# RenYurui/Global-Flow-Local-Attention

Hardware: AMD Instinct MI355X
Metric: images/sec (fwd+bwd) PoseGenerator 256x176 attn_layer=2,3 -- feature-warping hot path (higher is better)
Workload: dtype f32 (FC products: 2-term f16 splits exact to 2^-24 on f16 MFMA, f32 accumulate)

## Files before the change

global_flow_local_attention_amd/csrc/patch_mfma.hip:

```cpp
#include "gfla_common.h"
#include "patch_mfma.h"
#include "rs_taps.h"

namespace gfla {

typedef float pm_f32x16 __attribute__((ext_vector_type(16)));

struct PatchEntry {
  int q;
  float v;
};

constexpr int kPmStatSlots = 32;
constexpr int kPmTile = 32;
constexpr int kPmSub = 8;
constexpr int kPmChannels = 128;
constexpr int kPmMaxNB = 6;
constexpr int kPmGPitch = 33;

struct PmLayout {
  int64_t ntiles, table_bytes, rows_bytes, total;
};
static PmLayout pm_layout(int64_t B, int64_t HW, int entries) {
  PmLayout L;
  L.ntiles = ceil_div(HW, kPmTile);
  L.table_bytes = ((B * L.ntiles * kPmTile * entries * (int64_t)sizeof(PatchEntry)) + 255) & ~(int64_t)255;
  L.rows_bytes = ((B * L.ntiles * (int64_t)sizeof(int2)) + 255) & ~(int64_t)255;
  L.total = L.table_bytes + L.rows_bytes + 256;
  return L;
}

__device__ __forceinline__ unsigned pm_stat_total(const unsigned *stat) {
  unsigned tot = 0;
#pragma unroll
  for (int i = 0; i < kPmStatSlots; ++i) tot += stat[i];
  return tot;
}

__device__ __forceinline__ int pm_safe_int(float v) {
  return (int)fminf(fmaxf(v, -1048576.f), 1048576.f);
}

__device__ __forceinline__ void pm_store_tile_rows(int lo, int hi, int2 *slot, unsigned *stat) {
  __shared__ int s_lo[4], s_hi[4];
#pragma unroll
  for (int m = 32; m >= 1; m >>= 1) {
    lo = min(lo, __shfl_xor(lo, m));
    hi = max(hi, __shfl_xor(hi, m));
  }
  if ((threadIdx.x & 63) == 0) {
    s_lo[threadIdx.x >> 6] = lo;
    s_hi[threadIdx.x >> 6] = hi;
  }
  __syncthreads();
  if (threadIdx.x == 0) {
    const int l = min(min(s_lo[0], s_lo[1]), min(s_lo[2], s_lo[3])), h = max(max(s_hi[0], s_hi[1]), max(s_hi[2], s_hi[3]));
    *slot = make_int2(l, h);
    if (h >= l) atomicAdd(stat + (blockIdx.x + blockIdx.y * gridDim.x) % kPmStatSlots, (unsigned)(h - l + 1));
  }
}

struct Fold {
  int r_lo, r_hi, s_lo, s_hi, ty, tx;
  bool canonical;
};
__device__ __forceinline__ Fold pm_fold(int r, int s, int y0, int x0, int P, int Hs, int Ws) {
  Fold f;
  const int yy = y0 + r, xx = x0 + s;
  f.r_lo = f.r_hi = r;
  f.s_lo = f.s_hi = s;
  f.canonical = true;
  if (yy <= 0) {
    f.r_lo = 0;
    f.canonical = f.canonical && (yy == 0 || r == P - 1);
  } else if (yy >= Hs - 1) {
    f.r_hi = P - 1;
    f.canonical = f.canonical && (yy == Hs - 1 || r == 0);
  }
  if (xx <= 0) {
    f.s_lo = 0;
    f.canonical = f.canonical && (xx == 0 || s == P - 1);
  } else if (xx >= Ws - 1) {
    f.s_hi = P - 1;
    f.canonical = f.canonical && (xx == Ws - 1 || s == 0);
  }
  f.ty = clampi(yy, 0, Hs - 1);
  f.tx = clampi(xx, 0, Ws - 1);
  return f;
}

template <int K>
struct AggTaps {
  float fx0, fy0;
  int xf, yf, x0, y0;
  bool dense;
  __device__ __forceinline__ float dx(int t) const { return (fx0 + (float)(t - K / 2)) + (float)xf; }
  __device__ __forceinline__ float dy(int t) const { return (fy0 + (float)(t - K / 2)) + (float)yf; }
  __device__ __forceinline__ float ax(int t) const { const float d = dx(t); return d - floorf(d); }
  __device__ __forceinline__ float ay(int t) const { const float d = dy(t); return d - floorf(d); }
  __device__ __forceinline__ void init(float fx, float fy, int x, int y) {
    fx0 = fx, fy0 = fy, xf = x, yf = y;
    dense = true;
    x0 = y0 = 0;
#pragma unroll
    for (int t = 0; t < K; ++t) {
      const int ix = (int)floorf(dx(t)), iy = (int)floorf(dy(t));
      if (t == 0) x0 = ix, y0 = iy;
      dense = dense && (ix == x0 + t) && (iy == y0 + t);
    }
  }
};

template <int K>
__global__ __launch_bounds__(256) void agg_patch_table_kernel(const float *__restrict__ flow,
                                                             const float *__restrict__ attn,
                                                             PatchEntry *__restrict__ table,
                                                             int2 *__restrict__ tile_rows,
                                                             unsigned *__restrict__ stat, int H, int W, int Hs, int Ws,
                                                             int ntiles) {
  constexpr int P = K + 1, E = P * P, KK = K * K;
  static_assert(E % 2 == 0, "entries are written two at a time");
  typedef int i32x4 __attribute__((ext_vector_type(4)));
  const int64_t b = blockIdx.y;
  const int HW = H * W;
  const int tile = blockIdx.x * 8 + (threadIdx.x >> 5), pl = threadIdx.x & 31;
  if (tile >= ntiles) return;
  const int p = tile * kPmTile + pl;
  const float inv_kk = 1.f / (float)KK;
  int lo = 0x7fffffff, hi = -1;
  i32x4 *out = reinterpret_cast<i32x4 *>(table + ((b * ntiles + tile) * kPmTile + pl) * (int64_t)E);
  bool dense = false;
  AggTaps<K> tp;
  if (p < HW) {
    const int yf = p / W, xf = p - yf * W;
    tp.init(flow[(b * 2 + 0) * HW + p], flow[(b * 2 + 1) * HW + p], xf, yf);
    dense = tp.dense;
  }
  if (dense) {
    const int y0 = pm_safe_int((float)tp.y0), x0 = pm_safe_int((float)tp.x0);
    lo = clampi(y0, 0, Hs - 1);
    hi = clampi(y0 + K, 0, Hs - 1);
    float a[KK];
    const float *at = attn + b * (int64_t)KK * HW + p;
#pragma unroll
    for (int t = 0; t < KK; ++t) a[t] = at[(int64_t)t * HW] * inv_kk;
    float ax[K], ay[K];
#pragma unroll
    for (int t = 0; t < K; ++t) {
      ax[t] = tp.ax(t);
      ay[t] = tp.ay(t);
    }
    float v[P][P];
#pragma unroll
    for (int r = 0; r < P; ++r) {
#pragma unroll
      for (int q = 0; q < P; ++q) v[r][q] = 0.f;
#pragma unroll
      for (int j = 0; j < K; ++j) {
        float wrow = 0.f;
        if (r < K) wrow += a[r * K + j] * (1.f - ay[r]);
        if (r > 0) wrow += a[(r - 1) * K + j] * ay[r - 1];
        v[r][j] += wrow * (1.f - ax[j]);
        v[r][j + 1] += wrow * ax[j];
      }
    }
    int clo[P], chi[P], rlo[P], rhi[P], tx[P], ty[P];
    bool ccan[P], rcan[P];
#pragma unroll
    for (int i = 0; i < P; ++i) {
      const int xx = x0 + i, yy = y0 + i;
      clo[i] = chi[i] = rlo[i] = rhi[i] = i;
      ccan[i] = rcan[i] = true;
      if (xx <= 0) {
        clo[i] = 0;
        ccan[i] = xx == 0 || i == P - 1;
      } else if (xx >= Ws - 1) {
        chi[i] = P - 1;
        ccan[i] = xx == Ws - 1 || i == 0;
      }
      if (yy <= 0) {
        rlo[i] = 0;
        rcan[i] = yy == 0 || i == P - 1;
      } else if (yy >= Hs - 1) {
        rhi[i] = P - 1;
        rcan[i] = yy == Hs - 1 || i == 0;
      }
      tx[i] = clampi(xx, 0, Ws - 1);
      ty[i] = clampi(yy, 0, Hs - 1);
    }
    float cf[P][P];
#pragma unroll
    for (int r = 0; r < P; ++r)
#pragma unroll
      for (int q = 0; q < P; ++q) {
        float acc = 0.f;
#pragma unroll
        for (int q2 = 0; q2 < P; ++q2) acc += (q2 >= clo[q] && q2 <= chi[q]) ? v[r][q2] : 0.f;
        cf[r][q] = acc;
      }
#pragma unroll
    for (int r = 0; r < P; ++r)
#pragma unroll
      for (int q = 0; q < P; q += 2) {
        float acc0 = 0.f, acc1 = 0.f;
#pragma unroll
        for (int r2 = 0; r2 < P; ++r2) {
          const bool in = r2 >= rlo[r] && r2 <= rhi[r];
          acc0 += in ? cf[r2][q] : 0.f;
          acc1 += in ? cf[r2][q + 1] : 0.f;
        }
        const bool c0 = rcan[r] && ccan[q], c1 = rcan[r] && ccan[q + 1];
        i32x4 e;
        e.x = c0 ? (ty[r] << 16) | tx[q] : -1;
        e.y = c0 ? __float_as_int(acc0) : 0;
        e.z = c1 ? (ty[r] << 16) | tx[q + 1] : -1;
        e.w = c1 ? __float_as_int(acc1) : 0;
        out[(r * P + q) >> 1] = e;
      }
  } else {
    const i32x4 none = {-1, 0, -1, 0};
#pragma unroll
    for (int e = 0; e < E / 2; ++e) out[e] = none;
  }
#pragma unroll
  for (int msk = 16; msk >= 1; msk >>= 1) {
    lo = min(lo, __shfl_xor(lo, msk));
    hi = max(hi, __shfl_xor(hi, msk));
  }
  if (pl == 0) {
    tile_rows[b * ntiles + tile] = make_int2(lo, hi);
    if (hi >= lo) atomicAdd(stat + (tile + (int)b * ntiles) % kPmStatSlots, (unsigned)(hi - lo + 1));
  }
}

template <int K>
__global__ __launch_bounds__(256) void agg_scatter_nondense_kernel(const float *__restrict__ flow,
                                                                  const float *__restrict__ attn,
                                                                  const float *__restrict__ gout,
                                                                  float *__restrict__ gsrc, int C, int H, int W,
                                                                  int Hs, int Ws, const unsigned *__restrict__ stat,
                                                                  unsigned limit) {
  constexpr int KK = K * K;
  const int HW = H * W;
  if (pm_stat_total(stat) > limit) return;
  const int p = blockIdx.x * 256 + threadIdx.x;
  const int64_t b = blockIdx.y;
  if (p >= HW) return;
  const int yf = p / W, xf = p - yf * W;
  AggTaps<K> tp;
  tp.init(flow[(b * 2 + 0) * HW + p], flow[(b * 2 + 1) * HW + p], xf, yf);
  if (tp.dense) return;
  const float *at = attn + b * (int64_t)KK * HW + p;
  const float inv_kk = 1.f / (float)KK;
  for (int c = 0; c < C; ++c) {
    const float go = gout[(b * C + c) * (int64_t)HW + p] * inv_kk;
    float *gp = gsrc + (b * C + c) * (int64_t)Hs * Ws;
#pragma unroll 1
    for (int i = 0; i < K; ++i) {
      const float dy = tp.dy(i), fdy = floorf(dy);
      const int yT = clampi(pm_safe_int(fdy), 0, Hs - 1) * Ws, yB = clampi(pm_safe_int(fdy + 1), 0, Hs - 1) * Ws;
      const float yB_P = dy - fdy, yT_P = 1.f - yB_P;
#pragma unroll 1
      for (int j = 0; j < K; ++j) {
        const float dx = tp.dx(j), fdx = floorf(dx);
        const int xL = clampi(pm_safe_int(fdx), 0, Ws - 1), xR = clampi(pm_safe_int(fdx + 1), 0, Ws - 1);
        const float xR_P = dx - fdx, xL_P = 1.f - xR_P;
        const float gv = at[(int64_t)(i * K + j) * HW] * go;
        atomic_add(gp + yT + xL, gv * xL_P * yT_P);
        atomic_add(gp + yT + xR, gv * xR_P * yT_P);
        atomic_add(gp + yB + xL, gv * xL_P * yB_P);
        atomic_add(gp + yB + xR, gv * xR_P * yB_P);
      }
    }
  }
}

template <int KH>
__global__ __launch_bounds__(256) void rs_patch_table_kernel(const float *__restrict__ in2,
                                                            PatchEntry *__restrict__ table,
                                                            int2 *__restrict__ tile_rows,
                                                            unsigned *__restrict__ stat, int H, int W, int Hi, int Wi,
                                                            int trunc) {
  constexpr int P = 2 * KH, E = P * P;
  const int tile = blockIdx.x, ntiles = gridDim.x;
  const int64_t b = blockIdx.y;
  const int HW = H * W;
  const int pl = threadIdx.x >> 3, sub = threadIdx.x & (kPmSub - 1);
  const int p = tile * kPmTile + pl;
  PatchEntry *out = table + ((b * ntiles + tile) * kPmTile + pl) * (int64_t)E;
  int lo = 0x7fffffff, hi = -1;
  if (p < HW) {
    const int y = p / W, x = p - y * W;
    const float *i2 = in2 + b * 3 * (int64_t)HW + p;
    Taps<float, KH> t;
    t.template init<2>(i2[0], i2[HW], i2[2 * (int64_t)HW], x, y, Hi, Wi, 1, trunc != 0);
    const int y0 = pm_safe_int((float)t.iy0) - (KH - 1), x0 = pm_safe_int((float)t.ix0) - (KH - 1);
    lo = clampi(y0, 0, Hi - 1);
    hi = clampi(y0 + P - 1, 0, Hi - 1);
    float wy[P], wx[P];
#pragma unroll
    for (int r = 0; r < P; ++r) {
      wy[r] = (float)safe_div<float>(t.row_w(r), t.sum);
      wx[r] = t.col_w(r);
    }
    for (int e = sub; e < E; e += kPmSub) {
      const int r = e / P, s = e - r * P;
      const Fold f = pm_fold(r, s, y0, x0, P, Hi, Wi);
      float v = 0.f;
      if (f.canonical) {
#pragma unroll
        for (int rr = 0; rr < P; ++rr)
#pragma unroll
          for (int ss = 0; ss < P; ++ss)
            if (rr >= f.r_lo && rr <= f.r_hi && ss >= f.s_lo && ss <= f.s_hi) v += wy[rr] * wx[ss];
      }
      out[e] = f.canonical ? PatchEntry{(f.ty << 16) | f.tx, v} : PatchEntry{-1, 0.f};
    }
  } else {
    for (int e = sub; e < E; e += kPmSub) out[e] = PatchEntry{-1, 0.f};
  }
  pm_store_tile_rows(lo, hi, tile_rows + b * ntiles + tile, stat);
}

constexpr int kPmMaxEntriesPerThread = 5;

typedef float pm_f32x4 __attribute__((ext_vector_type(4)));

__device__ __forceinline__ void pm_fetch(pm_f32x4 (&gv)[4], int (&peq)[kPmMaxEntriesPerThread],
                                         float (&pev)[kPmMaxEntriesPerThread], int tile, const float *g_row, bool g_ok,
                                         bool g_vec, int gh, int HW, const PatchEntry *tab, int sub, int E) {
  const int pbase = tile * kPmTile + gh * 16;
#pragma unroll
  for (int q = 0; q < 4; ++q) {
    const int p = pbase + 4 * q;
    pm_f32x4 v = {0.f, 0.f, 0.f, 0.f};
    if (g_ok) {
      const float *src = g_row + (int64_t)tile * kPmTile + 4 * q;
      if (g_vec && p + 3 < HW) {
        v = *reinterpret_cast<const pm_f32x4 *>(src);
      } else {
        if (p < HW) v[0] = src[0];
        if (p + 1 < HW) v[1] = src[1];
        if (p + 2 < HW) v[2] = src[2];
        if (p + 3 < HW) v[3] = src[3];
      }
    }
    gv[q] = v;
  }
  const unsigned long long *tp = reinterpret_cast<const unsigned long long *>(tab + (int64_t)tile * kPmTile * E);
#pragma unroll
  for (int m = 0; m < kPmMaxEntriesPerThread; ++m) {
    const int e = sub + kPmSub * m;
    unsigned long long raw = 0xffffffffull;
    if (e < E) raw = tp[e];
    peq[m] = (int)(unsigned)(raw & 0xffffffffull);
    pev[m] = __uint_as_float((unsigned)(raw >> 32));
  }
}

template <int NB>
__global__ __launch_bounds__(256, 2) void patch_scatter_mfma_kernel(const float *__restrict__ G, float *__restrict__ dS,
                                                                   const PatchEntry *__restrict__ table,
                                                                   const int2 *__restrict__ tile_rows, int C, int HW,
                                                                   int Hs, int Ws, int R, int ntiles, int E,
                                                                   int accumulate, const unsigned *__restrict__ stat,
                                                                   unsigned limit) {
  constexpr int NQ = NB * 32;
  constexpr bool kSkip = NB >= 3;
  if (pm_stat_total(stat) > limit) return;
  extern __shared__ __attribute__((aligned(16))) unsigned char gfla_smem[];
  float *wt = reinterpret_cast<float *>(gfla_smem);
  float *gt = wt + kPmTile * NQ;
  unsigned short *list = reinterpret_cast<unsigned short *>(gt + kPmChannels * kPmGPitch);
  __shared__ int s_nlist;
  __shared__ unsigned s_mask[3];
  const int t = threadIdx.x, lane = t & 63, wave = t >> 6, l31 = lane & 31, kh = lane >> 5;
  const int band = blockIdx.x;
  const int64_t b = blockIdx.y;
  const int c0 = blockIdx.z * kPmChannels;
  const int by0 = band * R, by1 = min(Hs, by0 + R) - 1;
  const int nq = (by1 - by0 + 1) * Ws;

  if (wave == 0) {
    const int2 *tr = tile_rows + b * ntiles;
    int n = 0;
    for (int base = 0; base < ntiles; base += 64) {
      const int tile = base + lane;
      bool f = false;
      if (tile < ntiles) {
        const int2 rr = tr[tile];
        f = rr.x <= by1 && rr.y >= by0;
      }
      const unsigned long long m = __ballot(f);
      if (f) list[n + __popcll(m & ((1ull << lane) - 1ull))] = (unsigned short)tile;
      n += __popcll(m);
    }
    if (lane == 0) s_nlist = n;
  }
  __syncthreads();
  const int nlist = s_nlist;

  pm_f32x16 acc[NB];
#pragma unroll
  for (int j = 0; j < NB; ++j)
#pragma unroll
    for (int r = 0; r < 16; ++r) acc[j][r] = 0.f;

  const int gc = t >> 1, gh = t & 1;
  const bool g_ok = c0 + gc < C;
  const float *g_row = G + (b * C + (g_ok ? c0 + gc : 0)) * (int64_t)HW + gh * 16;
  const bool g_vec = (HW & 3) == 0 && (reinterpret_cast<uintptr_t>(G) & 15) == 0;
  const int pl = t >> 3, sub = t & (kPmSub - 1);
  const PatchEntry *tab = table + (b * ntiles * kPmTile + pl) * (int64_t)E;

  pm_f32x4 gv[4];
  int peq[kPmMaxEntriesPerThread];
  float pev[kPmMaxEntriesPerThread];
  if (nlist > 0) pm_fetch(gv, peq, pev, list[0], g_row, g_ok, g_vec, gh, HW, tab, sub, E);
  for (int li = 0; li < nlist; ++li) {
    __syncthreads();
#pragma unroll
    for (int i = 0; i < NB; ++i) reinterpret_cast<float4 *>(wt)[t + 256 * i] = make_float4(0.f, 0.f, 0.f, 0.f);
    if (kSkip && t < 3) s_mask[t] = 0u;
    {
      float *dst = gt + gc * kPmGPitch + gh * 16;
#pragma unroll
      for (int q = 0; q < 4; ++q) {
        dst[4 * q + 0] = gv[q][0];
        dst[4 * q + 1] = gv[q][1];
        dst[4 * q + 2] = gv[q][2];
        dst[4 * q + 3] = gv[q][3];
      }
    }
    __syncthreads();
    unsigned blocks = 0;
#pragma unroll
    for (int m = 0; m < kPmMaxEntriesPerThread; ++m) {
      const int q = peq[m];
      if (q >= 0) {
        const int ty = q >> 16, tx = q & 0xffff;
        if (ty >= by0 && ty <= by1) {
          const int col = (ty - by0) * Ws + tx;
          wt[pl * NQ + col] = pev[m];
          blocks |= 1u << (col >> 5);
        }
      }
    }
    if constexpr (kSkip) {
      blocks |= (unsigned)__shfl_xor((int)blocks, 1);
      blocks |= (unsigned)__shfl_xor((int)blocks, 2);
      blocks |= (unsigned)__shfl_xor((int)blocks, 4);
      blocks |= (unsigned)__shfl_xor((int)blocks, 8);
    }
    if (kSkip && (t & 15) == 0 && blocks) {
      const int base = (t >> 4) * NB, w = base >> 5, sh = base & 31;
      atomicOr(&s_mask[w], blocks << sh);
      if (sh + NB > 32) atomicOr(&s_mask[w + 1], blocks >> (32 - sh));
    }
    if (li + 1 < nlist)
      pm_fetch(gv, peq, pev, list[li + 1], g_row, g_ok, g_vec, gh, HW, tab, sub, E);
    __syncthreads();
    const unsigned mk0 = kSkip ? (unsigned)__builtin_amdgcn_readfirstlane((int)s_mask[0]) : 0xffffffffu;
    const unsigned mk1 = kSkip ? (unsigned)__builtin_amdgcn_readfirstlane((int)s_mask[1]) : 0xffffffffu;
    const unsigned mk2 = kSkip ? (unsigned)__builtin_amdgcn_readfirstlane((int)s_mask[2]) : 0xffffffffu;
    const float *ga = gt + (wave * 32 + l31) * kPmGPitch + kh;
    const float *wb = wt + kh * NQ + l31;
    float a = ga[0];
    float bq[NB];
#pragma unroll
    for (int j = 0; j < NB; ++j) bq[j] = wb[32 * j];
#pragma unroll 4
    for (int ks = 0; ks < kPmTile / 2; ++ks) {
      const float ac = a;
      float bc[NB];
#pragma unroll
      for (int j = 0; j < NB; ++j) bc[j] = bq[j];
      const int kn = ks + 1 < kPmTile / 2 ? ks + 1 : ks;
      a = ga[2 * kn];
#pragma unroll
      for (int j = 0; j < NB; ++j) bq[j] = wb[2 * kn * NQ + 32 * j];
      __builtin_amdgcn_sched_barrier(0);
#pragma unroll
      for (int j = 0; j < NB; ++j)
      {
        const int bit = ks * NB + j;
        const unsigned w = bit < 32 ? mk0 : (bit < 64 ? mk1 : mk2);
        if (!kSkip || ((w >> (bit & 31)) & 1u)) acc[j] = __builtin_amdgcn_mfma_f32_32x32x2f32(ac, bc[j], acc[j], 0, 0, 0);
      }
    }
  }
  const int64_t plane = (int64_t)Hs * Ws;
  const int cb = c0 + wave * 32 + 4 * kh;
  float *ob = dS + ((b * C + cb) * (int64_t)Hs + by0) * Ws + l31;
#pragma unroll
  for (int j = 0; j < NB; ++j) {
    const bool col_ok = 32 * j + l31 < nq;
    float oldv[16];
#pragma unroll
    for (int r = 0; r < 16; ++r) {
      const int dc = (r & 3) + 8 * (r >> 2);
      const bool ok = col_ok && cb + dc < C;
      oldv[r] = (accumulate && ok) ? ob[dc * plane + 32 * j] : 0.f;
    }
#pragma unroll
    for (int r = 0; r < 16; ++r) {
      const int dc = (r & 3) + 8 * (r >> 2);
      if (col_ok && cb + dc < C) ob[dc * plane + 32 * j] = oldv[r] + acc[j][r];
    }
  }
}

struct PmGeo {
  int R, NB, bands;
};
static PmGeo pm_geometry(int64_t B, int64_t C, int Hs, int Ws, int W, int patch) {
  (void)B, (void)C, (void)W, (void)patch;
  int R = tuning(GFLA_TUNE_PM_BAND_ROWS) > 0 ? tuning(GFLA_TUNE_PM_BAND_ROWS) : 96 / Ws;
  if (tuning(GFLA_TUNE_PM_BAND_ROWS) <= 0 && R < 2) R = (kPmMaxNB * 32) / Ws;
  if (R < 1) R = 1;
  if (R > Hs) R = Hs;
  while (R > 1 && R * Ws > kPmMaxNB * 32) --R;
  if (R * Ws > kPmMaxNB * 32) return PmGeo{0, 0, 0};
  return PmGeo{R, (int)ceil_div((int64_t)R * Ws, 32), (int)ceil_div(Hs, R)};
}

static bool pm_auto(bool aggregate, int64_t Ws) {
  if (tuning(GFLA_TUNE_PM) == 2) return true;
  return aggregate ? true : Ws <= 24;
}

static int64_t pm_lds_bytes(int NB, int64_t ntiles) {
  return (int64_t)(kPmTile * NB * 32 + kPmChannels * kPmGPitch) * (int64_t)sizeof(float) + ((ntiles + 7) & ~(int64_t)7) * 2;
}

static bool pm_supported(int64_t B, int64_t C, int64_t H, int64_t W, int64_t Hs, int64_t Ws) {
  if (!(B > 0 && B <= 65535 && C > 0 && Hs >= 2 && Ws >= 2 && Ws <= kPmMaxNB * 32 && Hs < 32768 && Ws < 32768 &&
        H * W <= (int64_t)kPmTile * 65535 && ceil_div(C, kPmChannels) <= 65535 && tuning(GFLA_TUNE_PM) != 1))
    return false;
  const PmGeo g = pm_geometry(B, C, (int)Hs, (int)Ws, (int)W, 0);
  return g.R > 0 && pm_lds_bytes(g.NB, ceil_div(H * W, kPmTile)) <= 64 * 1024;
}

static int pm_scatter(const float *G, float *dS, const PatchEntry *table, const int2 *tile_rows, int64_t B, int64_t C,
                      int64_t H, int64_t W, int64_t Hs, int64_t Ws, int entries, int patch, int accumulate,
                      const unsigned *stat, unsigned limit, hipStream_t stream) {
  const PmGeo g = pm_geometry(B, C, (int)Hs, (int)Ws, (int)W, patch);
  if (g.R == 0) return GFLA_ERR_UNSUPPORTED;
  const int ntiles = (int)ceil_div(H * W, kPmTile);
  const dim3 grid((unsigned)g.bands, (unsigned)B, (unsigned)ceil_div(C, kPmChannels));
  const unsigned lds = (unsigned)pm_lds_bytes(g.NB, ntiles);
  if (lds > 64 * 1024) return GFLA_ERR_UNSUPPORTED;
#define GFLA_PM(NB_)                                                                                              \
  case NB_:                                                                                                       \
    patch_scatter_mfma_kernel<NB_><<<grid, 256, lds, stream>>>(G, dS, table, tile_rows, (int)C, (int)(H * W), (int)Hs, \
                                                               (int)Ws, g.R, ntiles, entries, accumulate, stat, limit); \
    break
  switch (g.NB) {
    GFLA_PM(1);
    GFLA_PM(2);
    GFLA_PM(3);
    GFLA_PM(4);
    GFLA_PM(5);
    GFLA_PM(6);
    default: return GFLA_ERR_UNSUPPORTED;
  }
#undef GFLA_PM
  return launch_status();
}

static unsigned pm_limit(int64_t B, int64_t ntiles, int W, int patch, bool adaptive) {
  if (!adaptive || tuning(GFLA_TUNE_PM_LIMIT_ROWS) >= 100000) return 0xffffffffu;
  const double still = (double)kPmTile / W + 1.0 + patch;
  const double per_tile = tuning(GFLA_TUNE_PM_LIMIT_ROWS) > 0 ? (double)tuning(GFLA_TUNE_PM_LIMIT_ROWS) : 2.6 * still;
  const double total = per_tile * (double)B * (double)ntiles;
  return total >= 4.0e9 ? 0xffffffffu : (unsigned)total;
}

int agg_source_bwd_mfma(const float *flow, const float *attn, const float *gout, float *gsrc, void *workspace,
                        int64_t B, int64_t C, int64_t Hs, int64_t Ws, int64_t H, int64_t W, int k, int accumulate,
                        int adaptive, const unsigned **skip_stat, unsigned *skip_limit, hipStream_t stream) {
  if ((k != 3 && k != 5) || !pm_supported(B, C, H, W, Hs, Ws) || !workspace || !pm_auto(true, Ws)) return GFLA_ERR_UNSUPPORTED;
  const int entries = (k + 1) * (k + 1);
  const PmLayout L = pm_layout(B, H * W, entries);
  unsigned char *ws = static_cast<unsigned char *>(workspace);
  PatchEntry *table = reinterpret_cast<PatchEntry *>(ws);
  int2 *rows = reinterpret_cast<int2 *>(ws + L.table_bytes);
  unsigned *stat = reinterpret_cast<unsigned *>(ws + L.table_bytes + L.rows_bytes);
  const unsigned limit = pm_limit(B, L.ntiles, (int)W, k + 1, adaptive != 0);
  if (hipMemsetAsync(stat, 0, kPmStatSlots * 4, stream) != hipSuccess) return GFLA_ERR_LAUNCH;
  const dim3 tg((unsigned)ceil_div(L.ntiles, 8), (unsigned)B);
  if (k == 3)
    agg_patch_table_kernel<3><<<tg, 256, 0, stream>>>(flow, attn, table, rows, stat, (int)H, (int)W, (int)Hs, (int)Ws, (int)L.ntiles);
  else
    agg_patch_table_kernel<5><<<tg, 256, 0, stream>>>(flow, attn, table, rows, stat, (int)H, (int)W, (int)Hs, (int)Ws, (int)L.ntiles);
  int st = launch_status();
  if (st != GFLA_OK) return st;
  st = pm_scatter(gout, gsrc, table, rows, B, C, H, W, Hs, Ws, entries, k + 1, accumulate, stat, limit, stream);
  if (st != GFLA_OK) return st;
  const dim3 ng((unsigned)ceil_div(H * W, 256), (unsigned)B);
  if (k == 3)
    agg_scatter_nondense_kernel<3><<<ng, 256, 0, stream>>>(flow, attn, gout, gsrc, (int)C, (int)H, (int)W, (int)Hs, (int)Ws, stat, limit);
  else
    agg_scatter_nondense_kernel<5><<<ng, 256, 0, stream>>>(flow, attn, gout, gsrc, (int)C, (int)H, (int)W, (int)Hs, (int)Ws, stat, limit);
  if (skip_stat) *skip_stat = stat;
  if (skip_limit) *skip_limit = limit;
  return launch_status();
}

int rs_input1_bwd_mfma(const float *in2, const float *gout, float *gin1, void *workspace, int64_t B, int64_t C,
                       int64_t Hi, int64_t Wi, int64_t H, int64_t W, int k, int trunc, int accumulate, int adaptive,
                       const unsigned **skip_stat, unsigned *skip_limit, hipStream_t stream) {
  if ((k != 2 && k != 4) || !pm_supported(B, C, H, W, Hi, Wi) || !workspace || !pm_auto(false, Wi)) return GFLA_ERR_UNSUPPORTED;
  const int entries = k * k;
  const PmLayout L = pm_layout(B, H * W, entries);
  unsigned char *ws = static_cast<unsigned char *>(workspace);
  PatchEntry *table = reinterpret_cast<PatchEntry *>(ws);
  int2 *rows = reinterpret_cast<int2 *>(ws + L.table_bytes);
  unsigned *stat = reinterpret_cast<unsigned *>(ws + L.table_bytes + L.rows_bytes);
  const unsigned limit = pm_limit(B, L.ntiles, (int)W, k, adaptive != 0);
  if (hipMemsetAsync(stat, 0, kPmStatSlots * 4, stream) != hipSuccess) return GFLA_ERR_LAUNCH;
  const dim3 tg((unsigned)L.ntiles, (unsigned)B);
  if (k == 2)
    rs_patch_table_kernel<1><<<tg, 256, 0, stream>>>(in2, table, rows, stat, (int)H, (int)W, (int)Hi, (int)Wi, trunc);
  else
    rs_patch_table_kernel<2><<<tg, 256, 0, stream>>>(in2, table, rows, stat, (int)H, (int)W, (int)Hi, (int)Wi, trunc);
  const int st = launch_status();
  if (st != GFLA_OK) return st;
  if (skip_stat) *skip_stat = stat;
  if (skip_limit) *skip_limit = limit;
  return pm_scatter(gout, gin1, table, rows, B, C, H, W, Hi, Wi, entries, k, accumulate, stat, limit, stream);
}

int64_t pm_table_bytes(int64_t B, int64_t H, int64_t W, int entries) {
  if (B <= 0 || H <= 0 || W <= 0 || entries <= 0) return 0;
  return (pm_layout(B, H * W, entries).total + 255) & ~(int64_t)255;
}
int64_t pm_workspace_bytes(int64_t B, int64_t H, int64_t W, int entries) {
  if (B <= 0 || H <= 0 || W <= 0 || entries <= 0) return 0;
  return pm_table_bytes(B, H, W, entries) + B * H * W * kRsTapRecBytes;
}

}

extern "C" {
int64_t gfla_scatter_workspace_bytes(int64_t B, int64_t H, int64_t W, int patch_entries) {
  return gfla::pm_workspace_bytes(B, H, W, patch_entries);
}
}
```

Baseline: 10280.

## Retune patch-scatter MFMA kernel: occupancy, XCD remap, branchless fetches, split prefetch

Result: faster. 10390, median of 6 (+1.1%).

```diff
diff --git a/global_flow_local_attention_amd/csrc/patch_mfma.hip b/global_flow_local_attention_amd/csrc/patch_mfma.hip
--- a/global_flow_local_attention_amd/csrc/patch_mfma.hip
+++ b/global_flow_local_attention_amd/csrc/patch_mfma.hip
@@ -17,6 +17,7 @@
 constexpr int kPmChannels = 128;
 constexpr int kPmMaxNB = 6;
 constexpr int kPmGPitch = 33;
+constexpr int kPmEntrySlots = 40;
 
 struct PmLayout {
   int64_t ntiles, table_bytes, rows_bytes, total;
@@ -24,7 +25,7 @@
 static PmLayout pm_layout(int64_t B, int64_t HW, int entries) {
   PmLayout L;
   L.ntiles = ceil_div(HW, kPmTile);
-  L.table_bytes = ((B * L.ntiles * kPmTile * entries * (int64_t)sizeof(PatchEntry)) + 255) & ~(int64_t)255;
+  L.table_bytes = (((B * L.ntiles * kPmTile * entries + kPmEntrySlots) * (int64_t)sizeof(PatchEntry)) + 255) & ~(int64_t)255;
   L.rows_bytes = ((B * L.ntiles * (int64_t)sizeof(int2)) + 255) & ~(int64_t)255;
   L.total = L.table_bytes + L.rows_bytes + 256;
   return L;
@@ -323,190 +324,34 @@
 }
 
 constexpr int kPmMaxEntriesPerThread = 5;
+constexpr int kPmListBatch = 4;
 
 typedef float pm_f32x4 __attribute__((ext_vector_type(4)));
 
-__device__ __forceinline__ void pm_fetch(pm_f32x4 (&gv)[4], int (&peq)[kPmMaxEntriesPerThread],
-                                         float (&pev)[kPmMaxEntriesPerThread], int tile, const float *g_row, bool g_ok,
-                                         bool g_vec, int gh, int HW, const PatchEntry *tab, int sub, int E) {
+template <bool VEC>
+__device__ __forceinline__ void pm_fetch_g(pm_f32x4 (&gv)[4], int tile, const float *g_chan, int gh, int HW) {
   const int pbase = tile * kPmTile + gh * 16;
 #pragma unroll
   for (int q = 0; q < 4; ++q) {
     const int p = pbase + 4 * q;
-    pm_f32x4 v = {0.f, 0.f, 0.f, 0.f};
-    if (g_ok) {
-      const float *src = g_row + (int64_t)tile * kPmTile + 4 * q;
-      if (g_vec && p + 3 < HW) {
-        v = *reinterpret_cast<const pm_f32x4 *>(src);
-      } else {
-        if (p < HW) v[0] = src[0];
-        if (p + 1 < HW) v[1] = src[1];
-        if (p + 2 < HW) v[2] = src[2];
-        if (p + 3 < HW) v[3] = src[3];
-      }
-    }
-    gv[q] = v;
-  }
-  const unsigned long long *tp = reinterpret_cast<const unsigned long long *>(tab + (int64_t)tile * kPmTile * E);
+    if constexpr (VEC) {
+      gv[q] = *reinterpret_cast<const pm_f32x4 *>(g_chan + min(p, HW - 4));
+    } else {
+#pragma unroll
+      for (int i = 0; i < 4; ++i) gv[q][i] = g_chan[min(p + i, HW - 1)];
+    }
+  }
+}
+
+static_assert(kPmMaxEntriesPerThread * kPmSub <= kPmEntrySlots, "the slack behind the patch table covers every slot read");
+__device__ __forceinline__ void pm_fetch_entries(int (&peq)[kPmMaxEntriesPerThread], float (&pev)[kPmMaxEntriesPerThread],
+                                                 int tile, const PatchEntry *tab, int sub, int E) {
+  const unsigned long long *tp = reinterpret_cast<const unsigned long long *>(tab + (int64_t)tile * kPmTile * E) + sub;
 #pragma unroll
   for (int m = 0; m < kPmMaxEntriesPerThread; ++m) {
-    const int e = sub + kPmSub * m;
-    unsigned long long raw = 0xffffffffull;
-    if (e < E) raw = tp[e];
+    const unsigned long long raw = tp[kPmSub * m];
     peq[m] = (int)(unsigned)(raw & 0xffffffffull);
     pev[m] = __uint_as_float((unsigned)(raw >> 32));
-  }
-}
-
-template <int NB>
-__global__ __launch_bounds__(256, 2) void patch_scatter_mfma_kernel(const float *__restrict__ G, float *__restrict__ dS,
-                                                                   const PatchEntry *__restrict__ table,
-                                                                   const int2 *__restrict__ tile_rows, int C, int HW,
-                                                                   int Hs, int Ws, int R, int ntiles, int E,
-                                                                   int accumulate, const unsigned *__restrict__ stat,
-                                                                   unsigned limit) {
-  constexpr int NQ = NB * 32;
-  constexpr bool kSkip = NB >= 3;
-  if (pm_stat_total(stat) > limit) return;
-  extern __shared__ __attribute__((aligned(16))) unsigned char gfla_smem[];
-  float *wt = reinterpret_cast<float *>(gfla_smem);
-  float *gt = wt + kPmTile * NQ;
-  unsigned short *list = reinterpret_cast<unsigned short *>(gt + kPmChannels * kPmGPitch);
-  __shared__ int s_nlist;
-  __shared__ unsigned s_mask[3];
-  const int t = threadIdx.x, lane = t & 63, wave = t >> 6, l31 = lane & 31, kh = lane >> 5;
-  const int band = blockIdx.x;
-  const int64_t b = blockIdx.y;
-  const int c0 = blockIdx.z * kPmChannels;
-  const int by0 = band * R, by1 = min(Hs, by0 + R) - 1;
-  const int nq = (by1 - by0 + 1) * Ws;
-
-  if (wave == 0) {
-    const int2 *tr = tile_rows + b * ntiles;
-    int n = 0;
-    for (int base = 0; base < ntiles; base += 64) {
-      const int tile = base + lane;
-      bool f = false;
-      if (tile < ntiles) {
-        const int2 rr = tr[tile];
-        f = rr.x <= by1 && rr.y >= by0;
-      }
-      const unsigned long long m = __ballot(f);
-      if (f) list[n + __popcll(m & ((1ull << lane) - 1ull))] = (unsigned short)tile;
-      n += __popcll(m);
-    }
-    if (lane == 0) s_nlist = n;
-  }
-  __syncthreads();
-  const int nlist = s_nlist;
-
-  pm_f32x16 acc[NB];
-#pragma unroll
-  for (int j = 0; j < NB; ++j)
-#pragma unroll
-    for (int r = 0; r < 16; ++r) acc[j][r] = 0.f;
-
-  const int gc = t >> 1, gh = t & 1;
-  const bool g_ok = c0 + gc < C;
-  const float *g_row = G + (b * C + (g_ok ? c0 + gc : 0)) * (int64_t)HW + gh * 16;
-  const bool g_vec = (HW & 3) == 0 && (reinterpret_cast<uintptr_t>(G) & 15) == 0;
-  const int pl = t >> 3, sub = t & (kPmSub - 1);
-  const PatchEntry *tab = table + (b * ntiles * kPmTile + pl) * (int64_t)E;
-
-  pm_f32x4 gv[4];
-  int peq[kPmMaxEntriesPerThread];
-  float pev[kPmMaxEntriesPerThread];
-  if (nlist > 0) pm_fetch(gv, peq, pev, list[0], g_row, g_ok, g_vec, gh, HW, tab, sub, E);
-  for (int li = 0; li < nlist; ++li) {
-    __syncthreads();
-#pragma unroll
-    for (int i = 0; i < NB; ++i) reinterpret_cast<float4 *>(wt)[t + 256 * i] = make_float4(0.f, 0.f, 0.f, 0.f);
-    if (kSkip && t < 3) s_mask[t] = 0u;
-    {
-      float *dst = gt + gc * kPmGPitch + gh * 16;
-#pragma unroll
-      for (int q = 0; q < 4; ++q) {
-        dst[4 * q + 0] = gv[q][0];
-        dst[4 * q + 1] = gv[q][1];
-        dst[4 * q + 2] = gv[q][2];
-        dst[4 * q + 3] = gv[q][3];
-      }
-    }
-    __syncthreads();
-    unsigned blocks = 0;
-#pragma unroll
-    for (int m = 0; m < kPmMaxEntriesPerThread; ++m) {
-      const int q = peq[m];
-      if (q >= 0) {
-        const int ty = q >> 16, tx = q & 0xffff;
-        if (ty >= by0 && ty <= by1) {
-          const int col = (ty - by0) * Ws + tx;
-          wt[pl * NQ + col] = pev[m];
-          blocks |= 1u << (col >> 5);
-        }
-      }
-    }
-    if constexpr (kSkip) {
-      blocks |= (unsigned)__shfl_xor((int)blocks, 1);
-      blocks |= (unsigned)__shfl_xor((int)blocks, 2);
-      blocks |= (unsigned)__shfl_xor((int)blocks, 4);
-      blocks |= (unsigned)__shfl_xor((int)blocks, 8);
-    }
-    if (kSkip && (t & 15) == 0 && blocks) {
-      const int base = (t >> 4) * NB, w = base >> 5, sh = base & 31;
-      atomicOr(&s_mask[w], blocks << sh);
-      if (sh + NB > 32) atomicOr(&s_mask[w + 1], blocks >> (32 - sh));
-    }
-    if (li + 1 < nlist)
-      pm_fetch(gv, peq, pev, list[li + 1], g_row, g_ok, g_vec, gh, HW, tab, sub, E);
-    __syncthreads();
-    const unsigned mk0 = kSkip ? (unsigned)__builtin_amdgcn_readfirstlane((int)s_mask[0]) : 0xffffffffu;
-    const unsigned mk1 = kSkip ? (unsigned)__builtin_amdgcn_readfirstlane((int)s_mask[1]) : 0xffffffffu;
-    const unsigned mk2 = kSkip ? (unsigned)__builtin_amdgcn_readfirstlane((int)s_mask[2]) : 0xffffffffu;
-    const float *ga = gt + (wave * 32 + l31) * kPmGPitch + kh;
-    const float *wb = wt + kh * NQ + l31;
-    float a = ga[0];
-    float bq[NB];
-#pragma unroll
-    for (int j = 0; j < NB; ++j) bq[j] = wb[32 * j];
-#pragma unroll 4
-    for (int ks = 0; ks < kPmTile / 2; ++ks) {
-      const float ac = a;
-      float bc[NB];
-#pragma unroll
-      for (int j = 0; j < NB; ++j) bc[j] = bq[j];
-      const int kn = ks + 1 < kPmTile / 2 ? ks + 1 : ks;
-      a = ga[2 * kn];
-#pragma unroll
-      for (int j = 0; j < NB; ++j) bq[j] = wb[2 * kn * NQ + 32 * j];
-      __builtin_amdgcn_sched_barrier(0);
-#pragma unroll
-      for (int j = 0; j < NB; ++j)
-      {
-        const int bit = ks * NB + j;
-        const unsigned w = bit < 32 ? mk0 : (bit < 64 ? mk1 : mk2);
-        if (!kSkip || ((w >> (bit & 31)) & 1u)) acc[j] = __builtin_amdgcn_mfma_f32_32x32x2f32(ac, bc[j], acc[j], 0, 0, 0);
-      }
-    }
-  }
-  const int64_t plane = (int64_t)Hs * Ws;
-  const int cb = c0 + wave * 32 + 4 * kh;
-  float *ob = dS + ((b * C + cb) * (int64_t)Hs + by0) * Ws + l31;
-#pragma unroll
-  for (int j = 0; j < NB; ++j) {
-    const bool col_ok = 32 * j + l31 < nq;
-    float oldv[16];
-#pragma unroll
-    for (int r = 0; r < 16; ++r) {
-      const int dc = (r & 3) + 8 * (r >> 2);
-      const bool ok = col_ok && cb + dc < C;
-      oldv[r] = (accumulate && ok) ? ob[dc * plane + 32 * j] : 0.f;
-    }
-#pragma unroll
-    for (int r = 0; r < 16; ++r) {
-      const int dc = (r & 3) + 8 * (r >> 2);
-      if (col_ok && cb + dc < C) ob[dc * plane + 32 * j] = oldv[r] + acc[j][r];
-    }
   }
 }
 
@@ -541,6 +386,180 @@
   return g.R > 0 && pm_lds_bytes(g.NB, ceil_div(H * W, kPmTile)) <= 64 * 1024;
 }
 
+static bool pm_g_vec(const float *G, int64_t HW) {
+  return (HW & 3) == 0 && (reinterpret_cast<uintptr_t>(G) & 15) == 0;
+}
+
+template <int NB, bool VEC>
+__global__ __launch_bounds__(256, NB <= 3 ? 4 : 3) void patch_scatter_mfma_kernel(
+    const float *__restrict__ G, float *__restrict__ dS, const PatchEntry *__restrict__ table,
+    const int2 *__restrict__ tile_rows, int C, int HW, int Hs, int Ws, int R, int ntiles, int E, int accumulate,
+    const unsigned *__restrict__ stat, unsigned limit) {
+  constexpr int NQ = NB * 32;
+  constexpr bool kSkip = NB >= 3;
+  if (pm_stat_total(stat) > limit) return;
+  extern __shared__ __attribute__((aligned(16))) unsigned char gfla_smem[];
+  float *wt = reinterpret_cast<float *>(gfla_smem);
+  float *gt = wt + kPmTile * NQ;
+  unsigned short *list = reinterpret_cast<unsigned short *>(gt + kPmChannels * kPmGPitch);
+  __shared__ int s_nlist;
+  __shared__ unsigned s_mask[3];
+  const int t = threadIdx.x, lane = t & 63, wave = t >> 6, l31 = lane & 31, kh = lane >> 5;
+  const unsigned nwg = gridDim.x * gridDim.y * gridDim.z, lin = blockIdx.x + gridDim.x * (blockIdx.y + gridDim.y * blockIdx.z);
+  const unsigned xq = nwg >> 3, xr = nwg & 7u, xcd = lin & 7u;
+  const unsigned id = (xcd < xr ? xcd * (xq + 1) : xr * (xq + 1) + (xcd - xr) * xq) + (lin >> 3);
+  const int band = (int)(id % gridDim.x);
+  const int64_t b = (id / gridDim.x) % gridDim.y;
+  const int c0 = (int)(id / (gridDim.x * gridDim.y)) * kPmChannels;
+  const int by0 = band * R, by1 = min(Hs, by0 + R) - 1;
+  const int nq = (by1 - by0 + 1) * Ws;
+
+  if (wave == 0) {
+    const int2 *tr = tile_rows + b * ntiles;
+    int n = 0;
+    for (int base = 0; base < ntiles; base += 64 * kPmListBatch) {
+      int2 rr[kPmListBatch];
+#pragma unroll
+      for (int u = 0; u < kPmListBatch; ++u) rr[u] = tr[min(base + 64 * u + lane, ntiles - 1)];
+#pragma unroll
+      for (int u = 0; u < kPmListBatch; ++u) {
+        const int tile = base + 64 * u + lane;
+        const bool f = tile < ntiles && rr[u].x <= by1 && rr[u].y >= by0;
+        const unsigned long long m = __ballot(f);
+        if (f) list[n + __popcll(m & ((1ull << lane) - 1ull))] = (unsigned short)tile;
+        n += __popcll(m);
+      }
+    }
+    if (lane == 0) s_nlist = n;
+  }
+  __syncthreads();
+  const int nlist = s_nlist;
+
+  pm_f32x16 acc[NB];
+#pragma unroll
+  for (int j = 0; j < NB; ++j)
+#pragma unroll
+    for (int r = 0; r < 16; ++r) acc[j][r] = 0.f;
+
+  const int gc = t >> 1, gh = t & 1;
+  const bool g_ok = c0 + gc < C;
+  const float *g_chan = G + (b * C + min(c0 + gc, C - 1)) * (int64_t)HW;
+  const int pl = t >> 3, sub = t & (kPmSub - 1);
+  const PatchEntry *tab = table + (b * ntiles * kPmTile + pl) * (int64_t)E;
+
+  pm_f32x4 gv[4];
+  int peq[kPmMaxEntriesPerThread];
+  float pev[kPmMaxEntriesPerThread];
+  int tile = nlist > 0 ? __builtin_amdgcn_readfirstlane((int)list[0]) : 0;
+  pm_fetch_g<VEC>(gv, tile, g_chan, gh, HW);
+  pm_fetch_entries(peq, pev, tile, tab, sub, E);
+  for (int li = 0; li < nlist; ++li) {
+    __syncthreads();
+#pragma unroll
+    for (int i = 0; i < NB; ++i) reinterpret_cast<float4 *>(wt)[t + 256 * i] = make_float4(0.f, 0.f, 0.f, 0.f);
+    if (kSkip && t < 3) s_mask[t] = 0u;
+    {
+      float *dst = gt + gc * kPmGPitch + gh * 16;
+      const int nvalid = g_ok ? HW - (tile * kPmTile + gh * 16) : 0;
+#pragma unroll
+      for (int q = 0; q < 4; ++q)
+#pragma unroll
+        for (int i = 0; i < 4; ++i) dst[4 * q + i] = 4 * q + i < nvalid ? gv[q][i] : 0.f;
+    }
+    tile = __builtin_amdgcn_readfirstlane((int)list[li + 1 < nlist ? li + 1 : li]);
+    pm_fetch_g<VEC>(gv, tile, g_chan, gh, HW);
+    __syncthreads();
+    unsigned blocks = 0;
+#pragma unroll
+    for (int m = 0; m < kPmMaxEntriesPerThread; ++m) {
+      const int q = sub + kPmSub * m < E ? peq[m] : -1;
+      if (q >= 0) {
+        const int ty = q >> 16, tx = q & 0xffff;
+        if (ty >= by0 && ty <= by1) {
+          const int col = (ty - by0) * Ws + tx;
+          wt[pl * NQ + col] = pev[m];
+          blocks |= 1u << (col >> 5);
+        }
+      }
+    }
+    pm_fetch_entries(peq, pev, tile, tab, sub, E);
+    if constexpr (kSkip) {
+      blocks |= (unsigned)__shfl_xor((int)blocks, 1);
+      blocks |= (unsigned)__shfl_xor((int)blocks, 2);
+      blocks |= (unsigned)__shfl_xor((int)blocks, 4);
+      blocks |= (unsigned)__shfl_xor((int)blocks, 8);
+    }
+    if (kSkip && (t & 15) == 0 && blocks) {
+      const int base = (t >> 4) * NB, w = base >> 5, sh = base & 31;
+      atomicOr(&s_mask[w], blocks << sh);
+      if (sh + NB > 32) atomicOr(&s_mask[w + 1], blocks >> (32 - sh));
+    }
+    __syncthreads();
+    const unsigned mk0 = kSkip ? (unsigned)__builtin_amdgcn_readfirstlane((int)s_mask[0]) : 0xffffffffu;
+    const unsigned mk1 = kSkip ? (unsigned)__builtin_amdgcn_readfirstlane((int)s_mask[1]) : 0xffffffffu;
+    const unsigned mk2 = kSkip ? (unsigned)__builtin_amdgcn_readfirstlane((int)s_mask[2]) : 0xffffffffu;
+    const float *ga = gt + (wave * 32 + l31) * kPmGPitch + kh;
+    const float *wb = wt + kh * NQ + l31;
+    float a = ga[0];
+    float bq[NB];
+#pragma unroll
+    for (int j = 0; j < NB; ++j) bq[j] = wb[32 * j];
+#pragma unroll 4
+    for (int ks = 0; ks < kPmTile / 2; ++ks) {
+      const float ac = a;
+      float bc[NB];
+#pragma unroll
+      for (int j = 0; j < NB; ++j) bc[j] = bq[j];
+      const int kn = ks + 1 < kPmTile / 2 ? ks + 1 : ks;
+      a = ga[2 * kn];
+#pragma unroll
+      for (int j = 0; j < NB; ++j) bq[j] = wb[2 * kn * NQ + 32 * j];
+      __builtin_amdgcn_sched_barrier(0);
+#pragma unroll
+      for (int j = 0; j < NB; ++j)
+      {
+        const int bit = ks * NB + j;
+        const unsigned w = bit < 32 ? mk0 : (bit < 64 ? mk1 : mk2);
+        if (!kSkip || ((w >> (bit & 31)) & 1u)) acc[j] = __builtin_amdgcn_mfma_f32_32x32x2f32(ac, bc[j], acc[j], 0, 0, 0);
+      }
+    }
+  }
+  const unsigned plane_b = (unsigned)(Hs * Ws) * 4u;
+  const int cb = c0 + wave * 32 + 4 * kh;
+  char *band0 = reinterpret_cast<char *>(dS + ((b * C + c0) * (int64_t)Hs + by0) * Ws);
+  const unsigned lane_b = (unsigned)(wave * 32 + 4 * kh) * plane_b + (unsigned)l31 * 4u;
+  if (accumulate) {
+#pragma unroll
+    for (int j = 0; j < NB; ++j) {
+      const bool col_ok = 32 * j + l31 < nq;
+      float oldv[16];
+#pragma unroll
+      for (int r = 0; r < 16; ++r) {
+        const int dc = (r & 3) + 8 * (r >> 2);
+        const unsigned off = (col_ok && cb + dc < C) ? lane_b + (unsigned)dc * plane_b + 128u * j : 0u;
+        oldv[r] = *reinterpret_cast<const float *>(band0 + off);
+      }
+#pragma unroll
+      for (int r = 0; r < 16; ++r) {
+        const int dc = (r & 3) + 8 * (r >> 2);
+        if (col_ok && cb + dc < C)
+          *reinterpret_cast<float *>(band0 + (lane_b + (unsigned)dc * plane_b + 128u * j)) = oldv[r] + acc[j][r];
+      }
+    }
+  } else {
+#pragma unroll
+    for (int j = 0; j < NB; ++j) {
+      const bool col_ok = 32 * j + l31 < nq;
+#pragma unroll
+      for (int r = 0; r < 16; ++r) {
+        const int dc = (r & 3) + 8 * (r >> 2);
+        if (col_ok && cb + dc < C)
+          *reinterpret_cast<float *>(band0 + (lane_b + (unsigned)dc * plane_b + 128u * j)) = 0.f + acc[j][r];
+      }
+    }
+  }
+}
+
 static int pm_scatter(const float *G, float *dS, const PatchEntry *table, const int2 *tile_rows, int64_t B, int64_t C,
                       int64_t H, int64_t W, int64_t Hs, int64_t Ws, int entries, int patch, int accumulate,
                       const unsigned *stat, unsigned limit, hipStream_t stream) {
@@ -550,10 +569,16 @@
   const dim3 grid((unsigned)g.bands, (unsigned)B, (unsigned)ceil_div(C, kPmChannels));
   const unsigned lds = (unsigned)pm_lds_bytes(g.NB, ntiles);
   if (lds > 64 * 1024) return GFLA_ERR_UNSUPPORTED;
-#define GFLA_PM(NB_)                                                                                              \
-  case NB_:                                                                                                       \
-    patch_scatter_mfma_kernel<NB_><<<grid, 256, lds, stream>>>(G, dS, table, tile_rows, (int)C, (int)(H * W), (int)Hs, \
-                                                               (int)Ws, g.R, ntiles, entries, accumulate, stat, limit); \
+  const bool g_vec = pm_g_vec(G, H * W);
+#define GFLA_PM_LAUNCH(NB_, VEC_)                                                                                     \
+  patch_scatter_mfma_kernel<NB_, VEC_><<<grid, 256, lds, stream>>>(G, dS, table, tile_rows, (int)C, (int)(H * W), (int)Hs, \
+                                                                   (int)Ws, g.R, ntiles, entries, accumulate, stat, limit)
+#define GFLA_PM(NB_)                  \
+  case NB_:                           \
+    if (g_vec)                        \
+      GFLA_PM_LAUNCH(NB_, true);      \
+    else                              \
+      GFLA_PM_LAUNCH(NB_, false);     \
     break
   switch (g.NB) {
     GFLA_PM(1);
@@ -565,6 +590,7 @@
     default: return GFLA_ERR_UNSUPPORTED;
   }
 #undef GFLA_PM
+#undef GFLA_PM_LAUNCH
   return launch_status();
 }
 
```
